# waiwera/waiwera

Hardware: AMD Instinct MI355X
Metric: Newton steps/sec, 10M-cell eos_we (BCSR SpMV GB/s in roofline) (higher is better)
Workload: dtype f64

## Files before the change

waiwera_amd/csrc/capi.hip:

```cpp
#include "host.hpp"

using namespace wai;

namespace wai {

int fetch_flags(wai_ctx* c, int out[4]) {
  if (c->comm && c->comm->nranks > 1) {
    HIPCHK(c, hipMemcpyAsync(c->h_flags, c->d_flags, 4 * sizeof(int), hipMemcpyDeviceToHost, c->stream));
    HIPCHK(c, hipStreamSynchronize(c->stream));
    double v[4] = {(double)c->h_flags[0], -(double)c->h_flags[1], (double)c->h_flags[2], (double)c->h_flags[3]};
    HIPCHK(c, hipMemcpyAsync(c->d_red + 2048, v, sizeof(v), hipMemcpyHostToDevice, c->stream));
    if (comm_allreduce(c->comm, c->d_red + 2048, 4, 1, c->stream, c->err)) return -1;
    HIPCHK(c, hipMemcpyAsync(c->h_red + 8, c->d_red + 2048, sizeof(v), hipMemcpyDeviceToHost, c->stream));
    HIPCHK(c, hipStreamSynchronize(c->stream));
    out[0] = (int)c->h_red[8]; out[1] = c->h_flags[1]; out[2] = (int)c->h_red[10]; out[3] = (int)c->h_red[11];
  } else {
    HIPCHK(c, hipMemcpyAsync(c->h_flags, c->d_flags, 4 * sizeof(int), hipMemcpyDeviceToHost, c->stream));
    HIPCHK(c, hipStreamSynchronize(c->stream));
    for (int i = 0; i < 4; i++) out[i] = c->h_flags[i];
  }
  HIPCHK(c, hipMemcpyAsync(c->d_flags, FLAGS_RESET, sizeof(FLAGS_RESET), hipMemcpyHostToDevice, c->stream));
  return 0;
}

// ... 41 lines not shown
  if (allreduce_scal(c, S_W2, 1)) return -1;
  if (read_scal(c, S_W2, 1)) return -1;
  *out = std::sqrt(c->ks.h_scal[S_W2]);
  return 0;
}

int do_max_scaled(wai_ctx* c, const double* v, const double* scale, double tol, double* val, int* idx) {
  if (launch_max_scaled(c, v, scale, tol, val, idx)) return -1;
  if (c->comm && c->comm->nranks > 1) {
    HIPCHK(c, hipMemcpyAsync(c->d_red + 2048, val, sizeof(double), hipMemcpyHostToDevice, c->stream));
    if (comm_allreduce(c->comm, c->d_red + 2048, 1, 1, c->stream, c->err)) return -1;
    HIPCHK(c, hipMemcpyAsync(val, c->d_red + 2048, sizeof(double), hipMemcpyDeviceToHost, c->stream));
    HIPCHK(c, hipStreamSynchronize(c->stream));
  }
  return 0;
}

int snes_convergence(wai_ctx* c, int it, const double* f, const double* lhs_old, const double* y,
                     const double* update, double fnorm, double* max_residual, int* reason) {
  int loc;
  if (do_max_scaled(c, f, lhs_old, c->opts.ftol_abs, max_residual, &loc)) return -1;
  int r = 0;
  if (std::isnan(fnorm)) r = -4;
  else if (it == 0) { if (fnorm < 1.e-50) r = 3; }
  else if (fnorm <= 1.e-8 * c->fnorm0) r = 4;
  else if (fnorm > 1.e8 * c->fnorm0) r = -9;
  if (it < c->opts.min_newton_its) r = 0;
  else if (*max_residual < c->opts.ftol_rel) r = 1;
  else if (it > 0) {
    double mu;
    if (do_max_scaled(c, update, y, c->opts.utol_abs, &mu, &loc)) return -1;
    if (mu <= c->opts.utol_rel) r = 2;
  }
  *reason = r;
  return 0;
}

int do_newton_step(wai_ctx* c, double dt, int iter, double* y, const double* lhs_old, double* f,
                   int* ksp_its, int* reason, double* max_residual) {
  const int n = c->flow.n;
  *ksp_its = 0;
  if (iter == 0 && do_norm2(c, f, &c->fnorm0)) return -1;
  static_assert(F_REGION == F_T + 1 && F_OLD_REGION == F_T + 2, "the transition sweep's planes are consecutive");
  HIPCHK(c, hipMemcpyAsync(c->flu_last_iter + (size_t)F_T * c->mesh.n_local, c->flu + (size_t)F_T * c->mesh.n_local,
                           sizeof(double) * (size_t)3 * c->mesh.n_local, hipMemcpyDeviceToDevice, c->stream));
  c->last_iter_partial = true;
  int e = do_jacobian(c, dt, y, lhs_old);
  if (e < 0) return -1;
  if (e > 0) { *reason = -3; return 0; }
  int kreason = 0;
  double rn = 0.0;
  if (do_ksp(c, c->flow, f, c->w_delta, ksp_its, &kreason, &rn)) return -1;
  if (kreason < 0) { *reason = -3; return 0; }
  vec_copy(c, c->w_yold, y, c->flow.nl);
  vec_waxpy(c, y, -1.0, c->w_delta, c->w_yold, n);
  {
    Prof p(c, KC_TRANSITIONS);
    launch_transitions(c, c->w_yold, c->w_delta, y);
  }
  int fl[4];
  if (fetch_flags(c, fl)) return -1;
  if (fl[0]) { *reason = -3; return 0; }
  if (iter < c->opts.max_newton_its - 1) {
    e = do_residual(c, dt, y, lhs_old, f);
    if (e < 0) return -1;
    if (e > 0) { *reason = -3; return 0; }
  }
  double fnorm;
  if (do_norm2(c, f, &fnorm)) return -1;
  if (snes_convergence(c, iter + 1, f, lhs_old, y, c->w_delta, fnorm, max_residual, reason)) return -1;
  if (!*reason && iter + 1 >= c->opts.max_newton_its) *reason = -5;
  return 0;
}

int snapshot_step(wai_ctx* c) {
  HIPCHK(c, hipMemcpyAsync(c->flu_last_step, c->flu, sizeof(double) * (size_t)c->df * c->mesh.n_local,
                           hipMemcpyDeviceToDevice, c->stream));
  return 0;
}
int restore_step(wai_ctx* c) {
  HIPCHK(c, hipMemcpyAsync(c->flu, c->flu_last_step, sizeof(double) * (size_t)c->df * c->mesh.n_local,
                           hipMemcpyDeviceToDevice, c->stream));
  return 0;
}

}

extern "C" {

int wai_get_fluxes(wai_ctx* c, double* out) {
  if (!c || !out) return -2;
  const size_t n = (size_t)c->mesh.n_faces * (c->np + c->nmob);
  if (!n) return 0;
  DevBuf<double> tmp;
  if (tmp.alloc(c, n)) return -1;
  launch_face_fluxes(c, c->mesh.face_cells, tmp);
  HIPCHK(c, hipMemcpyAsync(out, tmp, n * sizeof(double), hipMemcpyDefault, c->stream));
  HIPCHK(c, hipStreamSynchronize(c->stream));
  return 0;
}
int wai_num_flux_dof(wai_ctx* c) { return c ? c->np + c->nmob : -2; }

int wai_get_fluid(wai_ctx* c, int which, double* out) {
  if (!c || !out) return -2;
  if (which == 1 && c->last_iter_partial) {
    c->err = "wai_get_fluid(1): the last-iteration record is partial after wai_newton_step (temperature, region, old region); "
             "call wai_pre_iteration for the whole record";
    return -2;
// ... 286 lines not shown
```

waiwera_amd/csrc/context.hpp:

```cpp
#pragma once
#include <hip/hip_runtime.h>
#include <string>
#include <type_traits>
#include <vector>
#include "../../include/waiwera_hip.h"
#include "colour_order.hpp"
#include "coupling_batch.hpp"
#include "devbuf.hpp"
#include "ilu_schedule.hpp"
#include "mesh_pattern.hpp"
#include "network_pass.hpp"
#include "network_wave.hpp"
#include "physics.hip.h"
#include "tile_schedule.hpp"

namespace wai {

__host__ __device__ __forceinline__ size_t ell_ld(size_t n) {
  size_t ld = (n + 511) & ~(size_t)511;
  if ((ld & 262143) == 0) ld += 512;
  return ld;
}
__host__ __device__ __forceinline__ size_t ell_rows(int bs, size_t n) {
  if (bs >= 3) return ell_ld(n);
// ... 432 lines not shown
int launch_coupling_batch(wai_ctx* c, const CouplingBatch& b, int col0, int ncol, double dt, const double* y, const double* lhs_old,
                          long long* launches, bool wave);
int launch_tracer_pick(wai_ctx* c, const double* X, int it, double* x);
int launch_tracer_put(wai_ctx* c, const double* x, int it, double* X);
int launch_tracer_alx(wai_ctx* c, const double* X, double* alx);
int launch_max_scaled(wai_ctx* c, const double* v, const double* scale, double tol, double* val,
                      int* idx);
int launch_fluid_aos(wai_ctx* c, const double* flu_soa, double* out_aos);
int launch_region_get(wai_ctx* c, double* out);
int launch_region_set(wai_ctx* c, const double* in, int first, int count);

int launch_spmv(wai_ctx* c, const Bcsr& M, const double* x, double* y);
int launch_ilu_factor_on(wai_ctx* c, const Bcsr& M, IluSchedule& s);
int launch_pc_on(wai_ctx* c, const Bcsr& M, const IluSchedule& s, bool spmv, const double* in, double* z,
                 int dot_mode, const double* aux, const int* list = nullptr, int nrun = 0, const Fin* fin = nullptr,
                 const double* in2 = nullptr, const Bcsr* F = nullptr, const int* row_map = nullptr);
int pc_kernel_kind(const wai_ctx* c, const Bcsr& M, const IluSchedule& s);
bool pc_axpy_capable(const wai_ctx* c, const Bcsr& M);
bool pc_axpy_default(const wai_ctx* c, const Bcsr& M);
int launch_big_solve(wai_ctx* c, const Bcsr& M, const IluSchedule& s, double* z);
int launch_colour_factor(wai_ctx* c, const Bcsr& M, const ColourSchedule& k, IluSchedule& s);
int launch_colour_solve(wai_ctx* c, const Bcsr& M, const ColourSchedule& k, const IluSchedule& s, double* z);
bool pc_colour_serves(const wai_ctx* c, const Bcsr& M, const ColourSchedule& k, bool one_rank);
int launch_pc_colour(wai_ctx* c, const Bcsr& M, const ColourSchedule& k, const IluSchedule& s, bool spmv, const double* in, double* z,
                     int dot_mode, const double* aux, const Fin* fin = nullptr);
int launch_sublu_solve(wai_ctx* c, const Bcsr& M, const IluSchedule& s, double* z);
bool sublu_vector_in_lds(const IluSchedule& s, int bs);
int launch_asm_gather_matrix(wai_ctx* c, const Bcsr& M, const AsmSystem& a);
int launch_pack_rows(wai_ctx* c, const Bcsr& M);
int launch_unpack_rows(wai_ctx* c, const Bcsr& M, const AsmSystem& a);
int launch_asm_gather(wai_ctx* c, const AsmSystem& a, const double* r);
int launch_asm_scatter(wai_ctx* c, const AsmSystem& a, double* z);
int vec_dots(wai_ctx* c, const double* a1, const double* b1, int slot1, const double* a2, const double* b2,
             int slot2, int n);
int launch_pc(wai_ctx* c, const Bcsr& M, bool spmv, const double* in, double* z, int dot_mode, const double* aux,
              const int* list = nullptr, int nrun = 0, const Fin* fin = nullptr, const double* in2 = nullptr);
Fin make_fin(wai_ctx* c, int slot0, int nslots, int phase, bool post = false);
inline Fin make_fin_dots(wai_ctx* c, int dot_mode, int phase, bool post = false) {
  return make_fin(c, pc_dot_slot0(dot_mode), pc_dot_nslots(dot_mode), phase, post);
}
int launch_ell_to_bcsr(wai_ctx* c, const Bcsr& M, double* bcsr);
int launch_dg_spmv(wai_ctx* c, const Bcsr& M, const double* x, double* y);
int launch_dg_factor(wai_ctx* c, const Bcsr& M, IluSchedule& s);
int launch_dg_pc(wai_ctx* c, const Bcsr& M, const IluSchedule& s, bool spmv, const double* in, double* z, const int* list, int nrun);
int launch_dg_big_solve(wai_ctx* c, const Bcsr& M, const IluSchedule& s, double* z);
int launch_dg_to_bcsr(wai_ctx* c, const Bcsr& M, double* bcsr);
int launch_bcsr_to_ell(wai_ctx* c, const double* bcsr, const Bcsr& M);
int vec_finalize(wai_ctx* c, int nb, int slot0, int nslots, int phase);
int vec_dot(wai_ctx* c, const double* a, const double* b, int n, int slot);
int partials_clear(wai_ctx* c, int slot0, int nslots);
int vec_copy(wai_ctx* c, double* dst, const double* src, size_t n);
int vec_zero(wai_ctx* c, double* dst, size_t n);
int vec_waxpy(wai_ctx* c, double* w, double alpha, const double* x, const double* y, int n);
int bcgs_scalars(wai_ctx* c, int phase, bool post = false);
int bcgs_update_xrp_derive(wai_ctx* c, const KrylovVecs& k, int n);
int bcgs_post(wai_ctx* c, int seq);
void read_env(wai_ctx* c);
int test_drop_partials(wai_ctx* c, int n);
int bcgs_update_p(wai_ctx* c, const KrylovVecs& k, int n);
int bcgs_update_s(wai_ctx* c, const KrylovVecs& k, int n);
int bcgs_update_xr(wai_ctx* c, const KrylovVecs& k, int n, bool dots = true, int fin_phase = -2, bool post = false);
int bcgs_update_xrp(wai_ctx* c, const KrylovVecs& k, int n);
int pack_halo_axpy(wai_ctx* c, const double* a, const double* b, int dof, hipStream_t stream = nullptr);
int gmres_mdot(wai_ctx* c, const double* basis, size_t ld, int n, const double* w, int k);
int gmres_maxpy_norm(wai_ctx* c, const double* basis, size_t ld, int n, double* w, int k);
int gmres_scale_to(wai_ctx* c, double* dst, const double* src, int slot_norm2, int n);
int gmres_update_x(wai_ctx* c, const double* basis, size_t ld, int n, double* x, const double* ycoef_host, int k);
int pack_halo(wai_ctx* c, const double* vec, int dof, hipStream_t stream = nullptr);
int unpack_halo(wai_ctx* c, double* vec, int dof, hipStream_t stream = nullptr);
}
```

waiwera_amd/csrc/kernels_fused.hip:

```cpp
#include "pc_generic.hip.h"
#include "pc_wide.hip.h"
#include "pc_park.hip.h"
#include "pc_rows.hip.h"
#include "pc_wave.hip.h"
#include "pc_colour.hip.h"
#include "krylov_vec.hip.h"

namespace wai {

static inline int vgrid(int n) {
  int g = (n + TPB - 1) / TPB;
  return g > 1024 ? 1024 : (g < 1 ? 1 : g);
}

void read_env(wai_ctx* c) {
  c->env.fin_separate = getenv("WAI_FIN_SEPARATE") != nullptr;
  c->env.no_col16 = getenv("WAI_NO_COL16") != nullptr;
  c->env.scalar_kernels = getenv("WAI_BCGS_SCALAR_KERNELS") != nullptr;
  c->env.iluk_level_path = getenv("WAI_ILUK_LEVEL_PATH") != nullptr;
  c->env.asm_unfused = getenv("WAI_ASM_UNFUSED") != nullptr;
  c->env.no_desc_share = getenv("WAI_NO_DESC_SHARE") != nullptr;
  c->env.no_pack = getenv("WAI_NO_PACK") != nullptr;
  c->env.colour_sweeps = getenv("WAI_COLOUR_SWEEPS") != nullptr;
  const char* st = getenv("WAI_PARK_STAGE");
// ... 245 lines not shown
}

int launch_pc(wai_ctx* c, const Bcsr& M, bool spmv, const double* in, double* z, int dot_mode, const double* aux,
              const int* list, int nrun, const Fin* fin, const double* in2) {
  return launch_pc_on(c, M, c->ilu, spmv, in, z, dot_mode, aux, list, nrun, fin, in2);
}
Fin make_fin(wai_ctx* c, int slot0, int nslots, int phase, bool post) {
  Fin f;
  f.slot0 = slot0; f.nslots = nslots; f.phase = phase;
  f.scal = c->ks.scal; f.post = c->ks.d_post; f.part2 = c->ks.partials2;
  f.seq = post ? ++c->ks.seq : 0;
  return f;
}

int vec_finalize(wai_ctx* c, int nb, int slot0, int nslots, int phase) {
  const int T = nb > 256 ? 1024 : 256;
  c->ks.n_launch++;
  hipLaunchKernelGGL(k_finalize, 1, T, 0, c->stream, c->ks.partials, c->ks.nb_max, nb, slot0, nslots, c->ks.scal, phase);
  return 0;
}

int vec_dot(wai_ctx* c, const double* a, const double* b, int n, int slot) {
  const int g = vgrid(n);
  c->ks.n_launch++;
  hipLaunchKernelGGL(k_dot, g, TPB, 0, c->stream, a, b, n, c->ks.partials, c->ks.nb_max, slot);
  return vec_finalize(c, g, slot, 1, -1);
}
int vec_dots(wai_ctx* c, const double* a1, const double* b1, int slot1, const double* a2, const double* b2,
             int slot2, int n) {
  const int g = vgrid(n);
  c->ks.n_launch++;
  hipLaunchKernelGGL(k_dots, g, TPB, 0, c->stream, a1, b1, slot1, a2, b2, slot2, n, c->ks.partials, c->ks.nb_max);
  c->ks.nb_pc = g;
  return 0;
}
int partials_clear(wai_ctx* c, int slot0, int nslots) {
  const size_t tot = (size_t)nslots * std::max(c->ks.nb_max, (int)FIN_MAXF);
  c->ks.n_launch++;
  hipLaunchKernelGGL(k_partials_clear, (int)((tot + TPB - 1) / TPB), TPB, 0, c->stream, c->ks.partials, c->ks.partials2, c->ks.nb_max, slot0, nslots);
  return 0;
}
int vec_copy(wai_ctx* c, double* dst, const double* src, size_t n) {
  c->ks.n_copy++;
  return hipMemcpyAsync(dst, src, n * sizeof(double), hipMemcpyDeviceToDevice, c->stream) == hipSuccess ? 0 : -1;
}
int vec_zero(wai_ctx* c, double* dst, size_t n) {
  return hipMemsetAsync(dst, 0, n * sizeof(double), c->stream) == hipSuccess ? 0 : -1;
}
int vec_waxpy(wai_ctx* c, double* w, double alpha, const double* x, const double* y, int n) {
  c->ks.n_launch++;
  hipLaunchKernelGGL(k_waxpy, vgrid(n), TPB, 0, c->stream, w, alpha, x, y, n);
  return 0;
}
int bcgs_scalars(wai_ctx* c, int phase, bool post) {
  c->ks.n_launch++;
  hipLaunchKernelGGL(k_bcgs_scalars, 1, 64, 0, c->stream, c->ks.scal, phase, c->ks.d_post, post ? ++c->ks.seq : 0);
  return 0;
}
int test_drop_partials(wai_ctx* c, int n) {
  return hipMemcpyToSymbolAsync(HIP_SYMBOL(g_drop_partials), &n, sizeof(int), 0, hipMemcpyHostToDevice, c->stream) == hipSuccess &&
         hipStreamSynchronize(c->stream) == hipSuccess ? 0 : -1;
}
int bcgs_post(wai_ctx* c, int seq) {
  c->ks.n_launch++;
  hipLaunchKernelGGL(k_bcgs_scalars, 1, 64, 0, c->stream, c->ks.scal, -1, c->ks.d_post, seq);
  return 0;
}

int bcgs_update_p(wai_ctx* c, const KrylovVecs& k, int n) {
  c->ks.n_launch++;
  hipLaunchKernelGGL(k_bcgs_p, vgrid(n), TPB, 0, c->stream, k.P, k.R, k.V, n, c->ks.scal);
  return 0;
}
int bcgs_update_s(wai_ctx* c, const KrylovVecs& k, int n) {
  c->ks.n_launch++;
  hipLaunchKernelGGL(k_bcgs_s, vgrid(n), TPB, 0, c->stream, k.S, k.R, k.V, n, c->ks.scal);
  return 0;
}
int bcgs_update_xr(wai_ctx* c, const KrylovVecs& k, int n, bool dots, int fin_phase, bool post) {
  const int g = vgrid(n);
  Fin fin;
  if (dots && fin_phase >= -1) { fin = make_fin(c, S_DP2, 2, fin_phase, post); fin.count = g; fin.nb = g; fin.nf = fin_slices(g); }
  c->ks.n_launch++;
  if (dots && fin.count > 0 && c->env.fin_separate) {
    Fin none;
    hipLaunchKernelGGL(k_bcgs_xr<true>, g, TPB, 0, c->stream, k.X, k.R, k.P, k.S, k.T,
                       k.RP, n, c->ks.scal, c->ks.partials, c->ks.nb_max, none);
    c->ks.nblocks = g;
    vec_finalize(c, g, S_DP2, 2, fin_phase);
    if (fin.seq > 0) bcgs_post(c, fin.seq);
    return 0;
  }
  if (dots)
    hipLaunchKernelGGL(k_bcgs_xr<true>, g + (fin.count > 0 ? fin.nf : 0), TPB, 0, c->stream, k.X, k.R, k.P, k.S, k.T,
                       k.RP, n, c->ks.scal, c->ks.partials, c->ks.nb_max, fin);
  else
    hipLaunchKernelGGL(k_bcgs_xr<false>, g, TPB, 0, c->stream, k.X, k.R, k.P, k.S, k.T,
                       k.RP, n, c->ks.scal, c->ks.partials, c->ks.nb_max, fin);
  c->ks.nblocks = g;
  return 0;
}
int bcgs_update_xrp(wai_ctx* c, const KrylovVecs& k, int n) {
  c->ks.n_launch++;
  hipLaunchKernelGGL(k_bcgs_xrp<false>, vgrid(n), TPB, 0, c->stream, k.X, k.R, k.P, k.V, k.T, n,
                     c->ks.scal, nullptr, nullptr, 0);
  return 0;
// ... 65 lines not shown
```

waiwera_amd/csrc/kernels_jacobian.hip:

```cpp
#include "assembly_device.hip.h"

namespace wai {

template <int KIND>
__global__ __launch_bounds__(TPB) void k_jacobian(MeshView m, const double* __restrict__ flu,
                                                  size_t stride, const double* __restrict__ flu_pert,
                                                  const double* __restrict__ hstep, int n_prim,
                                                  ResForm rf, double* __restrict__ val) {
  using E = EosT<KIND>;
  constexpr int np = E::np, bb = E::np * E::np;
  const int c = xcd_cell(m.n_owned);
  if (c < 0) return;
  CellState<KIND> own0;
  RockState rown;
  load_state<KIND>(flu, stride, c, own0);
  load_rock(m.rock, m.n_local, c, rown);
  const double vol = m.vol[c];
  double lold[np], lold2[np];
#pragma unroll
  for (int k = 0; k < np; k++) {
    lold[k] = rf.method == WAI_METHOD_DIRECTSS ? 0.0 : rf.last[(size_t)c * np + k];
    lold2[k] = rf.method == WAI_METHOD_BDF2 ? rf.last2[(size_t)c * np + k] : 0.0;
  }

// ... 206 lines not shown
  constexpr bool SHARE = np <= 2;
  const int c0 = c - (int)threadIdx.x, c1 = min(c0 + st, m.n_owned);
  if constexpr (SHARE) __syncthreads();
#pragma unroll 1
  for (int s = 0; s < m.max_deg; s++) {
    if (!((valid >> s) & 1u)) continue;
    const int blk = m.adj_blk[(size_t)s * m.n_owned + c];
    if (blk < 0) continue;
    const int fs = m.adj_face[(size_t)s * m.n_owned + c];
    const int o = m.adj_other[(size_t)s * m.n_owned + c];
    FaceGeom g;
    load_face(m, fs >> 1, g);
    RockState roth;
    load_rock(m.rock, m.n_local, o, roth);
#pragma unroll
    for (int k = 0; k < np; k++) {
      CellState<KIND> othk;
      if (SHARE && o >= c0 && o < c1) unpark_state<KIND>(park + (size_t)k * nld * st + (o - c0), st, othk);
      else load_state<KIND>(flu_pert + (size_t)k * E::df * n_prim, (size_t)n_prim, o, othk);
      double term[np], R[np];
      slot_term<KIND>(g, fs & 1, own0, rown, othk, roth, vol, term);
#pragma unroll
      for (int q = 0; q < np; q++) R[q] = 0.0;
#pragma unroll 1
      for (int s2 = 0; s2 < m.max_deg; s2++) {
        if ((valid >> s2) & 1u) {
#pragma unroll
          for (int q = 0; q < np; q++) R[q] += (s2 == s) ? term[q] : terms0[(size_t)(s2 * np + q) * st];
        }
      }
      const double h = hstep[(size_t)o * np + k];
#pragma unroll
      for (int r = 0; r < np; r++) {
        const double f1 = res_form(rf, L0[r], R[r] + src0[r], lold[r], lold2[r]);
        __builtin_nontemporal_store((f1 - f0[r]) / h, val + ell_ix(np, nrow, blk, r, k, (size_t)c));
      }
    }
  }
}

template <int KIND>
__device__ __forceinline__ void slot_flux(const FaceGeom& g, int side, const CellState<KIND>& own,
                                          const RockState& rown, const CellState<KIND>& oth,
                                          const RockState& roth, double* flux) {
  if (side == 0) face_flux<KIND>(g, own, rown, oth, roth, flux);
  else face_flux<KIND>(g, oth, roth, own, rown, flux);
}
__device__ __forceinline__ double res_dR(const ResForm& rf) {
  if (rf.method == WAI_METHOD_BDF2) return -rf.dt * (rf.ratio + 1.0);
  if (rf.method == WAI_METHOD_DIRECTSS) return 1.0;
  return -rf.dt;
}
constexpr int JSYM_WAVES = 2;
template <int KIND>
__global__ __launch_bounds__(ParkT<KIND>::threads, (EosT<KIND>::np <= 2 ? JSYM_WAVES : 1)) void k_jacobian_sym(MeshView m, const double* __restrict__ flu,
                                                  size_t stride, const double* __restrict__ flu_pert,
                                                  const double* __restrict__ hstep, int n_prim,
                                                  ResForm rf, double* __restrict__ val) {
  using E = EosT<KIND>;
  constexpr int np = E::np;
  const int c = xcd_cell(m.n_owned);
  if (c < 0) return;
  CellState<KIND> own0;
  RockState rown;
  load_state<KIND>(flu, stride, c, own0);
  load_rock(m.rock, m.n_local, c, rown);
  const double vol = m.vol[c];
  double hk[np];
#pragma unroll
  for (int k = 0; k < np; k++) hk[k] = hstep[(size_t)c * np + k];
  extern __shared__ double park[];
  constexpr int nld = ParkT<KIND>::npark;
  const int st = (int)blockDim.x;
  double Rk[np][np];
  double* lpark = park + (size_t)np * nld * st + threadIdx.x;
#pragma unroll
  for (int k = 0; k < np; k++) {
    CellState<KIND> ownk;
    double Lk[np];
    load_state<KIND>(flu_pert + (size_t)k * E::df * n_prim, (size_t)n_prim, c, ownk);
    cell_balance<KIND>(ownk, rown, Lk);
    park_state<KIND>(ownk, park + (size_t)k * nld * st + threadIdx.x, st);
#pragma unroll
    for (int q = 0; q < np; q++) { lpark[(size_t)(k * np + q) * st] = Lk[q]; Rk[k][q] = 0.0; }
  }
  const size_t nrow = m.n_owned;
  const double dR = res_dR(rf);
  double L0[np], R0[np], f0[np];
  cell_balance<KIND>(own0, rown, L0);
  bool ghost_cols = false;
#pragma unroll
  for (int k = 0; k < np; k++) R0[k] = 0.0;
#pragma unroll 1
  for (int s = 0; s < m.max_deg; s++) {
    const int fs = m.adj_face[(size_t)s * m.n_owned + c];
    if (fs < 0) continue;
    const int o = m.adj_other[(size_t)s * m.n_owned + c];
    const int tb = m.adj_tblk[(size_t)s * m.n_owned + c];
    FaceGeom g;
    load_face(m, fs >> 1, g);
    CellState<KIND> oth;
    RockState roth;
    load_state<KIND>(flu, stride, o, oth);
    load_rock_face(m.rock, m.n_local, o, g.dir, roth);
    const int side = fs & 1;
    const double sign = side ? 1.0 : -1.0;
    const double volo = tb >= 0 ? m.vol[o] : 1.0;
    double fl0[np], to0[np];
    slot_flux<KIND>(g, side, own0, rown, oth, roth, fl0);
#pragma unroll
    for (int q = 0; q < np; q++) {
      R0[q] += sign * (fl0[q] * g.area) / vol;
      to0[q] = -sign * (fl0[q] * g.area) / volo;
    }
#pragma unroll
    for (int k = 0; k < np; k++) {
      CellState<KIND> ownk;
      unpark_state<KIND>(park + (size_t)k * nld * st + threadIdx.x, st, ownk);
      double fl[np];
      slot_flux<KIND>(g, side, ownk, rown, oth, roth, fl);
#pragma unroll
      for (int q = 0; q < np; q++) Rk[k][q] += sign * (fl[q] * g.area) / vol;
      if (tb >= 0) {
#pragma unroll
        for (int r = 0; r < np; r++) {
          const double tok = -sign * (fl[r] * g.area) / volo;
          val[ell_ix(np, nrow, tb, r, k, (size_t)o)] = dR * (tok - to0[r]) / hk[k];
        }
      }
    }
    ghost_cols |= (m.adj_blk[(size_t)s * m.n_owned + c] >= 0 && o >= m.n_owned);
  }
  if (ghost_cols) {
#pragma unroll 1
    for (int s = 0; s < m.max_deg; s++) {
      const int fs = m.adj_face[(size_t)s * m.n_owned + c];
      if (fs < 0) continue;
      const int o = m.adj_other[(size_t)s * m.n_owned + c];
      const int blk = m.adj_blk[(size_t)s * m.n_owned + c];
      if (blk < 0 || o < m.n_owned) continue;
      FaceGeom g;
      load_face(m, fs >> 1, g);
      CellState<KIND> oth;
      RockState roth;
      load_state<KIND>(flu, stride, o, oth);
      load_rock_face(m.rock, m.n_local, o, g.dir, roth);
      const int side = fs & 1;
      const double sign = side ? 1.0 : -1.0;
      double fl0[np];
      slot_flux<KIND>(g, side, own0, rown, oth, roth, fl0);
#pragma unroll 1
      for (int k = 0; k < np; k++) {
        load_state<KIND>(flu_pert + (size_t)k * E::df * n_prim, (size_t)n_prim, o, oth);
        double fl[np];
        slot_flux<KIND>(g, side, own0, rown, oth, roth, fl);
        const double h = hstep[(size_t)o * np + k];
#pragma unroll
        for (int r = 0; r < np; r++) {
          const double t1 = sign * (fl[r] * g.area) / vol, t0 = sign * (fl0[r] * g.area) / vol;
          __builtin_nontemporal_store(dR * (t1 - t0) / h, val + ell_ix(np, nrow, blk, r, k, (size_t)c));
        }
      }
    }
  }
  double src0[np];
#pragma unroll
  for (int k = 0; k < np; k++) src0[k] = 0.0;
  source_terms<KIND>(m, c, own0, vol, src0);
  double lold[np], lold2[np];
#pragma unroll
  for (int k = 0; k < np; k++) {
    lold[k] = rf.method == WAI_METHOD_DIRECTSS ? 0.0 : rf.last[(size_t)c * np + k];
    lold2[k] = rf.method == WAI_METHOD_BDF2 ? rf.last2[(size_t)c * np + k] : 0.0;
  }
#pragma unroll
  for (int k = 0; k < np; k++) { R0[k] += src0[k]; f0[k] = res_form(rf, L0[k], R0[k], lold[k], lold2[k]); }
  const int dq = m.diag_blk[c];
#pragma unroll
  for (int k = 0; k < np; k++) {
    CellState<KIND> ownk;
    unpark_state<KIND>(park + (size_t)k * nld * st + threadIdx.x, st, ownk);
    source_terms<KIND>(m, c, ownk, vol, Rk[k]);
#pragma unroll
    for (int r = 0; r < np; r++) {
      const double f1 = res_form(rf, lpark[(size_t)(k * np + r) * st], Rk[k][r], lold[r], lold2[r]);
      __builtin_nontemporal_store((f1 - f0[r]) / hk[k], val + ell_ix(np, nrow, dq, r, k, (size_t)c));
    }
  }
}

int launch_jacobian(wai_ctx* c, double dt, const double* lhs_old) {
  const MeshView m = view(c);
  const size_t stride = c->mesh.n_local;
  const ResForm rf = res_form_of(c, dt, lhs_old);
  const char* ep = getenv("WAI_JAC_PARK");
  const bool park = !(ep && ep[0] == '0');
  const char* es = getenv("WAI_JAC_SYM");
  const bool sym = park && c->mesh.adj_tblk && (es ? es[0] == '1' : true);
  const char* kernel = nullptr;
  if (with_eos(c->kind, [&](auto k) {
        constexpr int K = decltype(k)::value;
        constexpr int T = ParkT<K>::threads;
        constexpr int sym_lds = EosT<K>::np * (ParkT<K>::npark + EosT<K>::np) * 8 * T;
        const int g = (((int)((m.n_owned + T - 1) / T) + 7) / 8) * 8;
        if (sym && (size_t)sym_lds <= c->lds_per_block) {
          kernel = "k_jacobian_sym";
          hipLaunchKernelGGL(k_jacobian_sym<K>, g, T, sym_lds, c->stream, m, c->flu, stride, c->flu_pert, c->hstep,
                             c->mesh.n_prim, rf, c->flow.A.val);
          return;
        }
        if (m.max_deg > MAXDEG) {
          c->err = "the row-wise Jacobian (WAI_JAC_SYM=0) supports cells with at most 8 faces; this mesh has a cell with " +
                   std::to_string(m.max_deg) + " (the default column-wise Jacobian takes up to 16)";
          return;
        }
        if (park && ParkT<K>::use) {
          kernel = "k_jacobian_park";
          hipLaunchKernelGGL(k_jacobian_park<K>, g, T, ParkT<K>::lds_bytes(m.max_deg), c->stream, m, c->flu, stride,
                             c->flu_pert, c->hstep, c->mesh.n_prim, rf, c->flow.A.val);
        } else {
          kernel = "k_jacobian";
          hipLaunchKernelGGL(k_jacobian<K>, grid8_for(m.n_owned), TPB, 0, c->stream, m, c->flu, stride, c->flu_pert, c->hstep,
                             c->mesh.n_prim, rf, c->flow.A.val);
        }
      })) return -1;
  return kernel ? launched(c, kernel) : -1;
}

}
```

waiwera_amd/csrc/krylov.hip:

```cpp
#include "host.hpp"

using namespace wai;

namespace wai {

int halo_exchange(wai_ctx* c, double* vec, int dof) {
  if (!c->comm || c->mesh.n_halo == 0) return 0;
  if (dof > c->max_dof_buf) { c->err = "halo dof too large"; return -1; }
  pack_halo(c, vec, dof);
  if (comm_exchange(c->comm, c->n_nbr, c->nbr_rank.data(), c->send_ptr.data(), c->recv_ptr.data(),
                    dof, c->d_sendbuf, c->d_recvbuf, c->stream, c->err))
    return -1;
  return unpack_halo(c, vec, dof);
}

int launch_pc_split(wai_ctx* c, const Bcsr& M, const double* x, double* z, int dot_mode, const double* aux, const Fin* fp, const double* x2,
                    hipEvent_t after) {
  const IluSchedule& s = c->ilu;
  if (launch_pc(c, M, true, x, z, dot_mode, aux, s.sub_int, s.n_int, nullptr, x2)) return -1;
  if (after) HIPCHK(c, hipStreamWaitEvent(c->stream, after, 0));
  return launch_pc(c, M, true, x, z, dot_mode, aux, s.sub_bnd, s.n_bnd, fp, x2);
}

int allreduce_scal(wai_ctx* c, int slot, int count) {
// ... 189 lines not shown
  BcgsPlan p;
  p.mode = bcgs_mode(c);
  p.fused3 = p.mode == 2; p.merged = p.mode >= 1;
  p.axpy = p.fused3 && pc_axpy_ok(c, sys);
  p.multi = c->comm && c->comm->nranks > 1;
  return p;
}
int bcgs_first_half(wai_ctx* c, LinSys& sys, const BcgsPlan& pl) {
  KrylovVecs& k = *sys.kv;
  if (!pl.fused3) { Prof p(c, KC_VECTOR); bcgs_update_p(c, k, sys.n); }
  if (int e = pc_amul(c, sys, k.P, k.V, PC_DOT_ZA, k.RP, pl.multi ? -1 : 2)) return e;
  Prof p(c, KC_VECTOR);
  if (pl.multi) {
    if (int e = allreduce_scal(c, S_D1, 1)) return e;
    if (pl.axpy && c->send_total > 0 && c->mesh.n_halo > 0 && !c->env.scalar_kernels) c->ks.alpha_pending = true;
    else bcgs_scalars(c, 2);
  }
  if (!pl.axpy) bcgs_update_s(c, k, sys.n);
  return 0;
}
int bcgs_second_half(wai_ctx* c, LinSys& sys, const BcgsPlan& pl) {
  KrylovVecs& k = *sys.kv;
  if (pl.fused3) {
    if (int e = pc_amul(c, sys, pl.axpy ? k.R : k.S, k.T, PC_DOT_MERGED, k.RP, pl.multi ? -1 : 6, pl.axpy ? k.V : nullptr, !pl.multi)) return e;
    Prof p(c, KC_VECTOR);
    if (pl.multi) {
      if (int e = allreduce_scal(c, S_D1, 5)) return e;
      if (c->env.scalar_kernels) { bcgs_scalars(c, 6, true); bcgs_update_xrp(c, k, sys.n); }
      else bcgs_update_xrp_derive(c, k, sys.n);
      return 0;
    }
    bcgs_update_xrp(c, k, sys.n);
    return 0;
  }
  if (int e = pc_amul(c, sys, k.S, k.T, pl.merged ? PC_DOT_MERGED : PC_DOT_XZ, pl.merged ? k.RP : nullptr, pl.merged ? -1 : 3)) return e;
  Prof p(c, KC_VECTOR);
  if (pl.merged) {
    if (pl.multi) { if (int e = allreduce_scal(c, S_D1, 5)) return e; }
    bcgs_scalars(c, 6, true);
    bcgs_update_xr(c, k, sys.n, false);
  } else {
    bcgs_update_xr(c, k, sys.n, true, 4, true);
  }
  return 0;
}

int ksp_bcgs(wai_ctx* c, LinSys& sys, const double* b, double* x, int* its, int* reason, double* rnorm) {
  KrylovVecs& k = *sys.kv;
  const int n = sys.n;
  const double rtol = sys.ksp.rtol, atol = sys.ksp.atol;
  const int maxits = sys.ksp.max_its;
  const BcgsPlan pl = bcgs_plan(c, sys);
  const bool multi = pl.multi;
  vec_zero(c, x, n);
  vec_zero(c, k.P, sys.nl);
  vec_zero(c, k.V, pl.fused3 ? sys.nl : n);
  c->ks.alpha_pending = false;
  partials_clear(c, S_D1, 5);
  vec_zero(c, c->ks.scal + S_BREAK, 1);
  {
    Prof p(c, KC_PC_APPLY);
    if (pc_solve(c, sys, b, k.R, PC_DOT_ZZ, nullptr, nullptr, multi ? -1 : 0)) return -1;
  }
  {
    Prof p(c, KC_VECTOR);
    if (multi) { if (allreduce_scal(c, S_DP2, 1)) return -1; bcgs_scalars(c, 0); }
    vec_copy(c, k.RP, k.R, n);
    if (pl.fused3) vec_copy(c, k.P, k.R, n);
  }
  if (read_scal(c, S_DP2, S_BREAK - S_DP2 + 1)) return -1;
  double dp = std::sqrt(c->ks.h_scal[S_DP2]);
  const double dp0 = dp, ttol = std::max(rtol * dp, atol);
  *its = 0;
  *reason = 0;
  if (c->ks.h_scal[S_BREAK] == 4.0) { *reason = -9; c->err = "a reduction's partial sum never arrived (finaliser wait ran out)"; }
  else if (std::isnan(dp)) *reason = -9;
  else if (dp <= ttol) *reason = (dp <= atol) ? 3 : 2;
  k.X = x;
  int rc = 0;
#ifdef WAI_BCGS_NO_SPECULATION
  const bool speculate = false;
#else
  const bool speculate = true;
#endif
  bool have_first_half = false;
  for (int i = 0; i < maxits && !*reason && !rc; i++) {
    if (!have_first_half && (rc = bcgs_first_half(c, sys, pl))) break;
    have_first_half = false;
    if ((rc = bcgs_second_half(c, sys, pl))) break;
    const int seq = c->ks.seq;
    if (speculate && i + 1 < maxits) {
      if ((rc = bcgs_first_half(c, sys, pl))) break;
      have_first_half = true;
    }
    if ((rc = wait_post(c, seq))) break;
    dp = std::sqrt(c->ks.h_scal[S_DP2]);
    *its = i + 1;
    const double brk = c->ks.h_scal[S_BREAK];
    if (brk == 4.0) { *reason = -9; c->err = "a reduction's partial sum never arrived (finaliser wait ran out)"; }
    else if (brk == 1.0) *reason = -5;
    else if (brk == 2.0) *reason = (dp == 0.0) ? 3 : -5;
    else if (std::isnan(dp)) *reason = -9;
    else if (dp <= ttol) *reason = (dp <= atol) ? 3 : 2;
    else if (brk == 3.0) *reason = -5;
    else if (dp >= 1.e4 * dp0) *reason = -4;
  }
  k.X = k.X_own;
  if (rc) return -1;
  if (!*reason) *reason = -3;
  *rnorm = dp;
  return 0;
}

int ksp_gmres(wai_ctx* c, LinSys& sys, const double* b, double* x, int* its, int* reason, double* rnorm) {
  KrylovVecs& k = *sys.kv;
  partials_clear(c, 0, NSLOTS);
  const int n = sys.n, m = std::min(std::max(sys.ksp.restart, 1), k.basis_m);
  const size_t ld = (size_t)sys.nl;
  const double rtol = sys.ksp.rtol, atol = sys.ksp.atol;
  const int maxits = sys.ksp.max_its;
  std::vector<double> H((size_t)(m + 1) * m, 0.0), cs(m), sn(m), g(m + 1), yv(m);
// ... 314 lines not shown
```

waiwera_amd/csrc/krylov_vec.hip.h:

```cpp
#pragma once
#include "reductions.hip.h"

namespace wai {


__global__ __launch_bounds__(TPB) void k_dot(const double* __restrict__ a, const double* __restrict__ b,
                                             int n, double* partials, int nb_max, int slot) {
  double v[1] = {0.0};
  for (int i = blockIdx.x * TPB + threadIdx.x; i < n; i += gridDim.x * TPB) v[0] += a[i] * b[i];
  const int slots[1] = {slot};
  block_reduce_store<1>(v, partials, nb_max, slots);
}

__global__ __launch_bounds__(1024) void k_finalize(const double* __restrict__ partials, int nb_max, int nb,
                                                   int slot0, int nslots, double* scal, int phase) {
  sum_partials(partials, nb_max, nb, slot0, nslots, scal, false);
  if (threadIdx.x == 0 && phase >= 0) derive_scalars(scal, phase);
}

__global__ __launch_bounds__(TPB) void k_partials_clear(double* partials, double* partials2, int nb_max, int slot0, int nslots) {
  const size_t i = (size_t)blockIdx.x * TPB + threadIdx.x;
  if (i < (size_t)nslots * nb_max) reinterpret_cast<unsigned long long*>(partials)[(size_t)slot0 * nb_max + i] = FIN_EMPTY;
  if (i < (size_t)nslots * FIN_MAXF) reinterpret_cast<unsigned long long*>(partials2)[(size_t)slot0 * FIN_MAXF + i] = FIN_EMPTY;
}
// ... 92 lines not shown
  auto one = [&](double x, double r0, double p, double v, double t, double& xo, double& ro, double& po) {
    const double si = __builtin_fma(nalpha, v, r0);
    xo = __builtin_fma(omega, si, __builtin_fma(alpha, p, x));
    ro = __builtin_fma(-omega, t, si);
    po = __builtin_fma(beta, p, __builtin_fma(ob, v, ro));
  };
  const int n2 = n >> 1;
  for (int i = blockIdx.x * TPB + threadIdx.x; i < n2; i += gridDim.x * TPB) {
    const wai_d2 x = __builtin_nontemporal_load(reinterpret_cast<const wai_d2*>(X) + i);
    const wai_d2 r0 = __builtin_nontemporal_load(reinterpret_cast<const wai_d2*>(R) + i);
    const wai_d2 p = __builtin_nontemporal_load(reinterpret_cast<const wai_d2*>(P) + i);
    const wai_d2 v = __builtin_nontemporal_load(reinterpret_cast<const wai_d2*>(V) + i);
    const wai_d2 t = __builtin_nontemporal_load(reinterpret_cast<const wai_d2*>(T) + i);
    wai_d2 xo, ro, po;
    double a, b, c2;
    one(x.x, r0.x, p.x, v.x, t.x, a, b, c2); xo.x = a; ro.x = b; po.x = c2;
    one(x.y, r0.y, p.y, v.y, t.y, a, b, c2); xo.y = a; ro.y = b; po.y = c2;
    __builtin_nontemporal_store(xo, reinterpret_cast<wai_d2*>(X) + i);
    __builtin_nontemporal_store(ro, reinterpret_cast<wai_d2*>(R) + i);
    __builtin_nontemporal_store(po, reinterpret_cast<wai_d2*>(P) + i);
  }
  if ((n & 1) && blockIdx.x == 0 && threadIdx.x == 0) {
    const int i = n - 1;
    double a, b, c2;
    one(X[i], R[i], P[i], V[i], T[i], a, b, c2);
    X[i] = a; R[i] = b; P[i] = c2;
  }
}

template <bool DERIVE>
__global__ __launch_bounds__(TPB) void k_pack_axpy(const double* __restrict__ a, const double* __restrict__ b,
                                                   double* s, const int* __restrict__ idx,
                                                   int n, int dof, double* __restrict__ buf) {
  const int t = blockIdx.x * TPB + threadIdx.x;
  double alpha;
  if constexpr (DERIVE) {
    const double d1 = s[S_D1];
    alpha = s[S_RHO] / d1;
    if (t == 0) {
      if (d1 == 0.0) s[S_BREAK] = 1.0;
      s[S_ALPHA] = alpha;
    }
  } else alpha = s[S_ALPHA];
  if (t >= n * dof) return;
  const int p = t / dof, k = t - p * dof;
  const size_t g = (size_t)idx[p] * dof + k;
  buf[t] = __builtin_fma(-alpha, b[g], a[g]);
}

__global__ __launch_bounds__(TPB) void k_waxpy(double* w, double alpha, const double* x, const double* y, int n) {
  for (int i = blockIdx.x * TPB + threadIdx.x; i < n; i += gridDim.x * TPB) w[i] = alpha * x[i] + y[i];
}

template <int CNT>
__global__ __launch_bounds__(TPB) void k_mdot(const double* __restrict__ w, const double* __restrict__ basis,
                                              size_t ld, int j0, int n, double* partials, int nb_max) {
  double v[CNT];
#pragma unroll
  for (int q = 0; q < CNT; q++) v[q] = 0.0;
  const size_t n2 = (size_t)n >> 1, stride = (size_t)gridDim.x * TPB;
  const wai_d2u* w2 = reinterpret_cast<const wai_d2u*>(w);
  auto one = [&](size_t i) {
    const wai_d2u wi = w2[i];
    wai_d2u b[CNT];
#pragma unroll
    for (int q = 0; q < CNT; q++) b[q] = __builtin_nontemporal_load(reinterpret_cast<const wai_d2u*>(basis + (size_t)(j0 + q) * ld) + i);
#pragma unroll
    for (int q = 0; q < CNT; q++) { v[q] += wi.x * b[q].x; v[q] += wi.y * b[q].y; }
  };
  size_t i = (size_t)blockIdx.x * TPB + threadIdx.x;
  for (; i + stride < n2; i += 2 * stride) { one(i); one(i + stride); }
  if (i < n2) one(i);
  if ((n & 1) && blockIdx.x == 0 && threadIdx.x == 0) {
#pragma unroll
    for (int q = 0; q < CNT; q++) v[q] += w[n - 1] * basis[(size_t)(j0 + q) * ld + n - 1];
  }
  int slots[CNT];
#pragma unroll
  for (int q = 0; q < CNT; q++) slots[q] = S_H + j0 + q;
  block_reduce_store<CNT>(v, partials, nb_max, slots);
}
__global__ __launch_bounds__(TPB) void k_maxpy_norm(double* __restrict__ w, const double* __restrict__ basis,
                                                    size_t ld, int k, int n, const double* __restrict__ s,
                                                    double* partials, int nb_max) {
  double v[1] = {0.0};
  const size_t n2 = (size_t)n >> 1, stride = (size_t)gridDim.x * TPB;
  wai_d2u* w2 = reinterpret_cast<wai_d2u*>(w);
  for (size_t i = (size_t)blockIdx.x * TPB + threadIdx.x; i < n2; i += stride) {
    wai_d2u wi = w2[i];
    int j = 0;
    for (; j + 8 <= k; j += 8) {
      wai_d2u b[8];
#pragma unroll
      for (int q = 0; q < 8; q++) b[q] = __builtin_nontemporal_load(reinterpret_cast<const wai_d2u*>(basis + (size_t)(j + q) * ld) + i);
#pragma unroll
      for (int q = 0; q < 8; q++) { const double h = s[S_H + j + q]; wi.x -= h * b[q].x; wi.y -= h * b[q].y; }
    }
    for (; j < k; j++) {
      const wai_d2u b = __builtin_nontemporal_load(reinterpret_cast<const wai_d2u*>(basis + (size_t)j * ld) + i);
      const double h = s[S_H + j];
      wi.x -= h * b.x; wi.y -= h * b.y;
    }
    w2[i] = wi;
    v[0] += wi.x * wi.x; v[0] += wi.y * wi.y;
  }
  if ((n & 1) && blockIdx.x == 0 && threadIdx.x == 0) {
// ... 45 lines not shown
```

Baseline: 5.323.

## Fuse Newton update copy+waxpy, pair Jacobian stores, trim BiCGStab preamble

Replaces the copy of y into yold and the following waxpy with one kernel that saves yold and updates y in a single pass. For 2x2 block equations of state, the symmetric Jacobian kernel now writes each block row as one 16-byte vector store instead of two scalar stores. The BiCGStab preamble drops a redundant zeroing of P and copies R into RP and P in one kernel. Each change cuts vector-sized memory passes or launches; each has an env switch to turn it off, and the paired store assumes block rows are contiguous and 16-byte aligned.

```diff
diff --git a/waiwera_amd/csrc/capi.hip b/waiwera_amd/csrc/capi.hip
--- a/waiwera_amd/csrc/capi.hip
+++ b/waiwera_amd/csrc/capi.hip
@@ -117,8 +117,13 @@
   double rn = 0.0;
   if (do_ksp(c, c->flow, f, c->w_delta, ksp_its, &kreason, &rn)) return -1;
   if (kreason < 0) { *reason = -3; return 0; }
-  vec_copy(c, c->w_yold, y, c->flow.nl);
-  vec_waxpy(c, y, -1.0, c->w_delta, c->w_yold, n);
+  const char* els = getenv("WAI_LINESEARCH_FUSE");
+  if (els && els[0] == '0') {
+    vec_copy(c, c->w_yold, y, c->flow.nl);
+    vec_waxpy(c, y, -1.0, c->w_delta, c->w_yold, n);
+  } else {
+    vec_keep_waxpy(c, y, c->w_yold, -1.0, c->w_delta, n, c->flow.nl);
+  }
   {
     Prof p(c, KC_TRANSITIONS);
     launch_transitions(c, c->w_yold, c->w_delta, y);
diff --git a/waiwera_amd/csrc/context.hpp b/waiwera_amd/csrc/context.hpp
--- a/waiwera_amd/csrc/context.hpp
+++ b/waiwera_amd/csrc/context.hpp
@@ -508,6 +508,8 @@
 int vec_copy(wai_ctx* c, double* dst, const double* src, size_t n);
 int vec_zero(wai_ctx* c, double* dst, size_t n);
 int vec_waxpy(wai_ctx* c, double* w, double alpha, const double* x, const double* y, int n);
+int vec_copy2(wai_ctx* c, double* a, double* b, const double* src, int n);
+int vec_keep_waxpy(wai_ctx* c, double* y, double* yold, double alpha, const double* delta, int n, int nl);
 int bcgs_scalars(wai_ctx* c, int phase, bool post = false);
 int bcgs_update_xrp_derive(wai_ctx* c, const KrylovVecs& k, int n);
 int bcgs_post(wai_ctx* c, int seq);
diff --git a/waiwera_amd/csrc/kernels_fused.hip b/waiwera_amd/csrc/kernels_fused.hip
--- a/waiwera_amd/csrc/kernels_fused.hip
+++ b/waiwera_amd/csrc/kernels_fused.hip
@@ -321,6 +321,16 @@
   hipLaunchKernelGGL(k_waxpy, vgrid(n), TPB, 0, c->stream, w, alpha, x, y, n);
   return 0;
 }
+int vec_copy2(wai_ctx* c, double* a, double* b, const double* src, int n) {
+  c->ks.n_launch++;
+  hipLaunchKernelGGL(k_copy2, vgrid(n), TPB, 0, c->stream, a, b, src, n);
+  return 0;
+}
+int vec_keep_waxpy(wai_ctx* c, double* y, double* yold, double alpha, const double* delta, int n, int nl) {
+  c->ks.n_launch++;
+  hipLaunchKernelGGL(k_keep_waxpy, vgrid(nl), TPB, 0, c->stream, y, yold, alpha, delta, n, nl);
+  return 0;
+}
 int bcgs_scalars(wai_ctx* c, int phase, bool post) {
   c->ks.n_launch++;
   hipLaunchKernelGGL(k_bcgs_scalars, 1, 64, 0, c->stream, c->ks.scal, phase, c->ks.d_post, post ? ++c->ks.seq : 0);
diff --git a/waiwera_amd/csrc/kernels_jacobian.hip b/waiwera_amd/csrc/kernels_jacobian.hip
--- a/waiwera_amd/csrc/kernels_jacobian.hip
+++ b/waiwera_amd/csrc/kernels_jacobian.hip
@@ -282,13 +282,15 @@
   return -rf.dt;
 }
 constexpr int JSYM_WAVES = 2;
-template <int KIND>
+typedef double jac_d2 __attribute__((ext_vector_type(2)));
+template <int KIND, bool PAIR>
 __global__ __launch_bounds__(ParkT<KIND>::threads, (EosT<KIND>::np <= 2 ? JSYM_WAVES : 1)) void k_jacobian_sym(MeshView m, const double* __restrict__ flu,
                                                   size_t stride, const double* __restrict__ flu_pert,
                                                   const double* __restrict__ hstep, int n_prim,
                                                   ResForm rf, double* __restrict__ val) {
   using E = EosT<KIND>;
   constexpr int np = E::np;
+  static_assert(!PAIR || np == 2, "16-byte block rows are the 2 x 2 layout's");
   const int c = xcd_cell(m.n_owned);
   if (c < 0) return;
   CellState<KIND> own0;
@@ -343,6 +345,7 @@
       R0[q] += sign * (fl0[q] * g.area) / vol;
       to0[q] = -sign * (fl0[q] * g.area) / volo;
     }
+    double col0[np];
 #pragma unroll
     for (int k = 0; k < np; k++) {
       CellState<KIND> ownk;
@@ -355,7 +358,16 @@
 #pragma unroll
         for (int r = 0; r < np; r++) {
           const double tok = -sign * (fl[r] * g.area) / volo;
-          val[ell_ix(np, nrow, tb, r, k, (size_t)o)] = dR * (tok - to0[r]) / hk[k];
+          const double v = dR * (tok - to0[r]) / hk[k];
+          if constexpr (PAIR) {
+            if (k == 0) col0[r] = v;
+            else {
+              jac_d2 pr; pr.x = col0[r]; pr.y = v;
+              *reinterpret_cast<jac_d2*>(val + ell_ix(np, nrow, tb, r, 0, (size_t)o)) = pr;
+            }
+          } else {
+            val[ell_ix(np, nrow, tb, r, k, (size_t)o)] = v;
+          }
         }
       }
     }
@@ -406,6 +418,7 @@
 #pragma unroll
   for (int k = 0; k < np; k++) { R0[k] += src0[k]; f0[k] = res_form(rf, L0[k], R0[k], lold[k], lold2[k]); }
   const int dq = m.diag_blk[c];
+  double col0[np];
 #pragma unroll
   for (int k = 0; k < np; k++) {
     CellState<KIND> ownk;
@@ -414,7 +427,16 @@
 #pragma unroll
     for (int r = 0; r < np; r++) {
       const double f1 = res_form(rf, lpark[(size_t)(k * np + r) * st], Rk[k][r], lold[r], lold2[r]);
-      __builtin_nontemporal_store((f1 - f0[r]) / hk[k], val + ell_ix(np, nrow, dq, r, k, (size_t)c));
+      const double v = (f1 - f0[r]) / hk[k];
+      if constexpr (PAIR) {
+        if (k == 0) col0[r] = v;
+        else {
+          jac_d2 pr; pr.x = col0[r]; pr.y = v;
+          __builtin_nontemporal_store(pr, reinterpret_cast<jac_d2*>(val + ell_ix(np, nrow, dq, r, 0, (size_t)c)));
+        }
+      } else {
+        __builtin_nontemporal_store(v, val + ell_ix(np, nrow, dq, r, k, (size_t)c));
+      }
     }
   }
 }
@@ -427,6 +449,8 @@
   const bool park = !(ep && ep[0] == '0');
   const char* es = getenv("WAI_JAC_SYM");
   const bool sym = park && c->mesh.adj_tblk && (es ? es[0] == '1' : true);
+  const char* eq = getenv("WAI_JAC_PAIR");
+  const bool pair = !(eq && eq[0] == '0');
   const char* kernel = nullptr;
   if (with_eos(c->kind, [&](auto k) {
         constexpr int K = decltype(k)::value;
@@ -435,8 +459,16 @@
         const int g = (((int)((m.n_owned + T - 1) / T) + 7) / 8) * 8;
         if (sym && (size_t)sym_lds <= c->lds_per_block) {
           kernel = "k_jacobian_sym";
-          hipLaunchKernelGGL(k_jacobian_sym<K>, g, T, sym_lds, c->stream, m, c->flu, stride, c->flu_pert, c->hstep,
-                             c->mesh.n_prim, rf, c->flow.A.val);
+          auto launch_sym = [&](auto pr) {
+            hipLaunchKernelGGL((k_jacobian_sym<K, decltype(pr)::value>), g, T, sym_lds, c->stream, m, c->flu, stride, c->flu_pert,
+                               c->hstep, c->mesh.n_prim, rf, c->flow.A.val);
+          };
+          if constexpr (EosT<K>::np == 2) {
+            if (pair) launch_sym(std::true_type{});
+            else launch_sym(std::false_type{});
+          } else {
+            launch_sym(std::false_type{});
+          }
           return;
         }
         if (m.max_deg > MAXDEG) {
diff --git a/waiwera_amd/csrc/krylov.hip b/waiwera_amd/csrc/krylov.hip
--- a/waiwera_amd/csrc/krylov.hip
+++ b/waiwera_amd/csrc/krylov.hip
@@ -265,8 +265,10 @@
   const int maxits = sys.ksp.max_its;
   const BcgsPlan pl = bcgs_plan(c, sys);
   const bool multi = pl.multi;
+  const char* epre = getenv("WAI_BCGS_PREAMBLE");
+  const bool lean = !(epre && epre[0] == '0');
   vec_zero(c, x, n);
-  vec_zero(c, k.P, sys.nl);
+  if (!(lean && pl.fused3 && sys.nl == n)) vec_zero(c, k.P, sys.nl);
   vec_zero(c, k.V, pl.fused3 ? sys.nl : n);
   c->ks.alpha_pending = false;
   partials_clear(c, S_D1, 5);
@@ -278,8 +280,11 @@
   {
     Prof p(c, KC_VECTOR);
     if (multi) { if (allreduce_scal(c, S_DP2, 1)) return -1; bcgs_scalars(c, 0); }
-    vec_copy(c, k.RP, k.R, n);
-    if (pl.fused3) vec_copy(c, k.P, k.R, n);
+    if (pl.fused3 && lean) vec_copy2(c, k.RP, k.P, k.R, n);
+    else {
+      vec_copy(c, k.RP, k.R, n);
+      if (pl.fused3) vec_copy(c, k.P, k.R, n);
+    }
   }
   if (read_scal(c, S_DP2, S_BREAK - S_DP2 + 1)) return -1;
   double dp = std::sqrt(c->ks.h_scal[S_DP2]);
diff --git a/waiwera_amd/csrc/krylov_vec.hip.h b/waiwera_amd/csrc/krylov_vec.hip.h
--- a/waiwera_amd/csrc/krylov_vec.hip.h
+++ b/waiwera_amd/csrc/krylov_vec.hip.h
@@ -168,6 +168,21 @@
   for (int i = blockIdx.x * TPB + threadIdx.x; i < n; i += gridDim.x * TPB) w[i] = alpha * x[i] + y[i];
 }
 
+__global__ __launch_bounds__(TPB) void k_copy2(double* __restrict__ a, double* __restrict__ b, const double* __restrict__ src, int n) {
+  for (int i = blockIdx.x * TPB + threadIdx.x; i < n; i += gridDim.x * TPB) {
+    const double v = ldv(src + i);
+    a[i] = v; b[i] = v;
+  }
+}
+__global__ __launch_bounds__(TPB) void k_keep_waxpy(double* __restrict__ y, double* __restrict__ yold, double alpha,
+                                                    const double* __restrict__ delta, int n, int nl) {
+  for (int i = blockIdx.x * TPB + threadIdx.x; i < nl; i += gridDim.x * TPB) {
+    const double yo = y[i];
+    yold[i] = yo;
+    if (i < n) y[i] = alpha * delta[i] + yo;
+  }
+}
+
 template <int CNT>
 __global__ __launch_bounds__(TPB) void k_mdot(const double* __restrict__ w, const double* __restrict__ basis,
                                               size_t ld, int j0, int n, double* partials, int nb_max) {
```

Result: no change. 5.309 (-0.3%).
